# bxh1/VIDO-SLAM

Measured on AMD Instinct MI355X. Metric: frames/sec end-to-end (flow+depth+track+local-BA) at 640x480; BA iters/sec, higher is better.
Workload: dtype f32

## Files before the change

### vido-slam_amd/csrc/convsmall.hip

```cpp
#include "common.hpp"

namespace {
template <int K>
__global__ __launch_bounds__(256) void k_conv_kxk_c2(const float* __restrict__ x, const float* __restrict__ w, const float* __restrict__ bias, const float* __restrict__ res,
                                                     float* __restrict__ y, int Cin, int H, int W)
{
    constexpr int R = K / 2, TS = 16 + K - 1, CC = 8, NT = CC * TS * TS, NL = (NT + 255) / 256, NW = (CC * K * K * 2 + 255) / 256;
    __shared__ float tile[NT];
    __shared__ __attribute__((aligned(8))) float wl[NW * 256];
    const int tid = threadIdx.x, tx = tid & 15, ty = tid >> 4, bx = blockIdx.x * 16, by = blockIdx.y * 16;
    const size_t HW = (size_t)H * W;
    int toff[NL]; bool tin[NL]; int tch[NL];
#pragma unroll
    for (int j = 0; j < NL; j++) {
        const int i = min(tid + 256 * j, NT - 1), c = i / (TS * TS), r = i - c * (TS * TS), yy = r / TS, xx = r - yy * TS, gy = by + yy - R, gx = bx + xx - R;
        tch[j] = c; tin[j] = tid + 256 * j < NT && gy >= 0 && gy < H && gx >= 0 && gx < W;
        toff[j] = min(max(gy, 0), H - 1) * W + min(max(gx, 0), W - 1);
    }
    float tv[NL], wv[NW];
    auto fetch = [&](int c0) {
#pragma unroll
        for (int j = 0; j < NL; j++) { const int c = min(c0 + tch[j], Cin - 1); tv[j] = x[(size_t)c * HW + toff[j]]; }
#pragma unroll
        for (int j = 0; j < NW; j++) {
            const int i = min(tid + 256 * j, CC * K * K * 2 - 1), o = i & 1, t = (i >> 1) % (K * K), c = min(c0 + (i >> 1) / (K * K), Cin - 1);
            wv[j] = w[((size_t)o * Cin + c) * (K * K) + t];
        }
    };
    float acc0 = bias ? bias[0] : 0.f, acc1 = bias ? bias[1] : 0.f;
    fetch(0);
    for (int c0 = 0; c0 < Cin; c0 += CC) {
        __syncthreads();
#pragma unroll
        for (int j = 0; j < NL; j++) if (tid + 256 * j < NT) tile[tid + 256 * j] = (tin[j] && c0 + tch[j] < Cin) ? tv[j] : 0.f;
#pragma unroll
        for (int j = 0; j < NW; j++) { const int i = tid + 256 * j; if (i < CC * K * K * 2) wl[i] = (c0 + (i >> 1) / (K * K) < Cin) ? wv[j] : 0.f; }
        __syncthreads();
        if (c0 + CC < Cin) fetch(c0 + CC);
#pragma unroll 2
        for (int c = 0; c < CC; c++) {
            const float* tc = tile + c * TS * TS + ty * TS + tx;
            const float2* wc = (const float2*)wl + c * K * K;
#pragma unroll
            for (int dy = 0; dy < K; dy++)
#pragma unroll
                for (int dx = 0; dx < K; dx++) {
                    const float v = tc[dy * TS + dx];
                    const float2 ww = wc[dy * K + dx];
                    acc0 = fmaf(v, ww.x, acc0); acc1 = fmaf(v, ww.y, acc1);
                }
        }
    }
    const int gy = by + ty, gx = bx + tx;
    if (gy < H && gx < W) {
        const size_t o = (size_t)gy * W + gx;
        y[o] = acc0 + (res ? res[o] : 0.f); y[HW + o] = acc1 + (res ? res[HW + o] : 0.f);
    }
}

typedef float f32x16s __attribute__((ext_vector_type(16)));
template <int CB, bool RES, int D>
__global__ __launch_bounds__(256) void k_conv1x1_skinny(const float* __restrict__ x, const float* __restrict__ wp, const float* __restrict__ bias, const float* __restrict__ res,
                                                        float* __restrict__ y, int Cin, int Cout, long long HW, float slope, unsigned xbytes, unsigned wbytes)
{
    const int lane = threadIdx.x & 63, wv = __builtin_amdgcn_readfirstlane(threadIdx.x >> 6);
    const long long p0 = ((long long)blockIdx.x * 4 + wv) * 32;
    if (p0 >= HW) return;
    const long long p = min(p0 + (lane & 31), HW - 1);
    const int nkp = Cin >> 1;
    f32x16s acc[CB];
#pragma unroll
    for (int cb = 0; cb < CB; cb++)
#pragma unroll
        for (int r = 0; r < 16; r++) acc[cb][r] = 0.f;
    const __amdgpu_buffer_rsrc_t xr = __builtin_amdgcn_make_buffer_rsrc((void*)x, 0, xbytes, 0x00020000);
    const __amdgpu_buffer_rsrc_t wr = __builtin_amdgcn_make_buffer_rsrc((void*)wp, 0, wbytes, 0x00020000);
    const unsigned xvo = 4u * (unsigned)((lane >> 5) * HW + p), wvo = 4u * (unsigned)lane;
    const unsigned hw8 = 8u * (unsigned)HW;
    float b[D], a[D][CB], bn[D], an[D][CB];
    auto fetch = [&](int kp0, float (&fb)[D], float (&fa)[D][CB]) {
#pragma unroll
        for (int u = 0; u < D; u++) {
            const int kp = min(kp0 + u, nkp - 1);
            fb[u] = __builtin_bit_cast(float, __builtin_amdgcn_raw_buffer_load_b32(xr, xvo, hw8 * (unsigned)kp, 0));
#pragma unroll
            for (int cb = 0; cb < CB; cb++) fa[u][cb] = __builtin_bit_cast(float, __builtin_amdgcn_raw_buffer_load_b32(wr, wvo, 256u * (unsigned)(cb * nkp + kp), 0));
        }
    };
    constexpr bool AHEAD = D > 4;
    if (AHEAD) fetch(0, b, a);
    for (int kp0 = 0; kp0 < nkp; kp0 += D) {
        if (!AHEAD) fetch(kp0, b, a);
        else if (kp0 + D < nkp) fetch(kp0 + D, bn, an);
#pragma unroll
        for (int u = 0; u < D; u++)
            if (kp0 + u < nkp) {
#pragma unroll
                for (int cb = 0; cb < CB; cb++) acc[cb] = __builtin_amdgcn_mfma_f32_32x32x2f32(a[u][cb], b[u], acc[cb], 0, 0, 0);
            }
        if (AHEAD) {
#pragma unroll
            for (int u = 0; u < D; u++) {
                b[u] = bn[u];
#pragma unroll
                for (int cb = 0; cb < CB; cb++) a[u][cb] = an[u][cb];
            }
        }
    }
    if (p0 + (lane & 31) < HW) {
#pragma unroll
        for (int cb = 0; cb < CB; cb++) {
            float bv[16], rv[16];
#pragma unroll
            for (int r = 0; r < 16; r++) {
                const int co = min(cb * 32 + 8 * (r >> 2) + 4 * (lane >> 5) + (r & 3), Cout - 1);
                bv[r] = bias ? bias[co] : 0.f; rv[r] = RES ? res[(size_t)co * HW + p] : 0.f;
            }
#pragma unroll
            for (int r = 0; r < 16; r++) {
                const int co = cb * 32 + 8 * (r >> 2) + 4 * (lane >> 5) + (r & 3);
                const float v = acc[cb][r] + bv[r] + rv[r];
                if (co < Cout) y[(size_t)co * HW + p] = fmaxf(v, v * slope);
            }
        }
    }
}
}

extern "C" {

int vido_conv_kxk_c2(vido_ctx* ctx, const float* x, const float* w, const float* bias, const float* residual, float* y, int cin, int k, int h, int wd)
{
    if (!ctx) return VIDO_E_INVALID;
    if (!x || !w || !y || x == y || cin < 1 || h < 1 || wd < 1 || (k != 3 && k != 5 && k != 7)) return vido_set_error(ctx, VIDO_E_INVALID, "conv_kxk_c2: bad arguments (k = %d)", k);
    HIP_TRY(ctx, hipSetDevice(ctx->device));
    hipStream_t st = ctx->has_ext_stream ? ctx->ext_stream : ctx->stream;
    const dim3 grid((wd + 15) / 16, (h + 15) / 16), blk(256);
    if (k == 7) hipLaunchKernelGGL(k_conv_kxk_c2<7>, grid, blk, 0, st, x, w, bias, residual, y, cin, h, wd);
    else if (k == 5) hipLaunchKernelGGL(k_conv_kxk_c2<5>, grid, blk, 0, st, x, w, bias, residual, y, cin, h, wd);
    else hipLaunchKernelGGL(k_conv_kxk_c2<3>, grid, blk, 0, st, x, w, bias, residual, y, cin, h, wd);
    HIP_TRY(ctx, hipGetLastError());
    return VIDO_OK;
}

int vido_conv1x1_skinny(vido_ctx* ctx, const float* x, const float* w_packed, const float* bias, const float* residual, float* y, int cin, int cout, long long hw, float slope)
{
    if (!ctx) return VIDO_E_INVALID;
    if (!x || !w_packed || !y || x == y || cin < 2 || (cin & 1) || cin > 256 || cout < 1 || cout > 256 || hw < 1 || slope < 0.f || slope > 1.f || 4ll * cin * hw >= (1ll << 32))
        return vido_set_error(ctx, VIDO_E_INVALID, "conv1x1_skinny: no kernel for %d -> %d channels", cin, cout);
    HIP_TRY(ctx, hipSetDevice(ctx->device));
    hipStream_t st = ctx->has_ext_stream ? ctx->ext_stream : ctx->stream;
    const dim3 grid((unsigned)((hw + 127) / 128)), blk(256);
    const int cbn = (cout + 31) / 32;
    const unsigned xb = (unsigned)(4ll * cin * hw), wb = (unsigned)(4ll * cbn * 32 * cin);
    int depth = 16;
    if (const char* e = getenv("VIDO_SKINNY_DEPTH")) {
        depth = atoi(e);
        if (depth != 4 && depth != 8 && depth != 16) return vido_set_error(ctx, VIDO_E_INVALID, "conv1x1_skinny: VIDO_SKINNY_DEPTH=%s (4, 8 or 16)", e);
    }
#define SK_LAUNCH(CBV, DV) { if (residual) hipLaunchKernelGGL((k_conv1x1_skinny<CBV, true, DV>), grid, blk, 0, st, x, w_packed, bias, residual, y, cin, cout, hw, slope, xb, wb); \
                             else hipLaunchKernelGGL((k_conv1x1_skinny<CBV, false, DV>), grid, blk, 0, st, x, w_packed, bias, residual, y, cin, cout, hw, slope, xb, wb); }
    switch (cbn) {
    case 1: if (depth == 4) SK_LAUNCH(1, 4) else if (depth == 8) SK_LAUNCH(1, 8) else SK_LAUNCH(1, 16) break;
    case 2: SK_LAUNCH(2, 4) break; case 3: SK_LAUNCH(3, 4) break; case 4: SK_LAUNCH(4, 4) break;
    case 5: SK_LAUNCH(5, 4) break; case 6: SK_LAUNCH(6, 4) break; case 7: SK_LAUNCH(7, 4) break; default: SK_LAUNCH(8, 4) break;
    }
#undef SK_LAUNCH
    HIP_TRY(ctx, hipGetLastError());
    return VIDO_OK;
}

}
```

Baseline: 134.8.

## Add strip-tiled 2-output KxK conv and LDS-staged weights for skinny 1x1 conv

Adds a new KxK two-output-channel conv kernel in which each thread computes P horizontal pixels. It stages 64/P input channels per pass in dynamic LDS and software-pipelines row loads through a register ring, reusing window values across neighbouring pixels to cut LDS traffic. The new kernel is the default, with P=2. The skinny 1x1 MFMA conv also gains a variant that copies packed weights into LDS, used for 2-4 output blocks when the weights fit in 32 KB. It also changes the default pipeline depth to 16 or 8 for the 3- and 4-block cases, at the cost of more LDS use and register pressure.

```diff
diff --git a/vido-slam_amd/csrc/convsmall.hip b/vido-slam_amd/csrc/convsmall.hip
--- a/vido-slam_amd/csrc/convsmall.hip
+++ b/vido-slam_amd/csrc/convsmall.hip
@@ -58,12 +58,137 @@
     }
 }
 
+template <int K, int P>
+__global__ __launch_bounds__(256) void k_conv_kxk_c2_strip(const float* __restrict__ x, const float* __restrict__ w, const float* __restrict__ bias, const float* __restrict__ res,
+                                                           float* __restrict__ y, int Cin, int H, int W)
+{
+    constexpr int R = K / 2, CC = 64 / P, TW = 16 * P, TSW = TW + K - 1, TSH = 16 + K - 1, NW = TSH * TSW, NS = (NW + 255) / 256, NP = NS * 256, NV = P + K - 1;
+    constexpr int NWT = CC * K * 16, NWL = (NWT + 255) / 256, K4 = (K + 3) / 4, NB = 4, UC = 4;
+    static_assert((UC * K) % NB == 0 && NB - 1 <= K, "ring position of a row is a constant");
+    static_assert(P % 2 == 0 && TSW % 2 == 0 && NV % 2 == 0, "8-byte window reads");
+    extern __shared__ __attribute__((aligned(16))) float tile_s[];
+    float* const wl = tile_s, * const tile = tile_s + NWT;
+    const int tid = threadIdx.x, tx = tid & 15, ty = tid >> 4, bx = blockIdx.x * TW, by = blockIdx.y * 16;
+    const size_t HW = (size_t)H * W;
+    unsigned toff[NS]; bool tin[NS];
+#pragma unroll
+    for (int s = 0; s < NS; s++) {
+        const int i = min(tid + 256 * s, NW - 1), yy = i / TSW, xx = i - yy * TSW, gy = by + yy - R, gx = bx + xx - R;
+        tin[s] = tid + 256 * s < NW && gy >= 0 && gy < H && gx >= 0 && gx < W;
+        toff[s] = (unsigned)(min(max(gy, 0), H - 1) * W + min(max(gx, 0), W - 1));
+    }
+    float tv[CC][NS], wv[NWL];
+    auto fetch = [&](int c0) {
+#pragma unroll
+        for (int j = 0; j < NWL; j++) {
+            const int i = min(tid + 256 * j, NWT - 1), dx = min(i & 7, K - 1), o = (i >> 3) & 1, r = i >> 4, c = min(c0 + r / K, Cin - 1), dy = r % K;
+            wv[j] = w[((size_t)o * Cin + c) * (K * K) + dy * K + dx];
+        }
+#pragma unroll
+        for (int c = 0; c < CC; c++) {
+            const float* xc = x + (size_t)min(c0 + c, Cin - 1) * HW;
+#pragma unroll
+            for (int s = 0; s < NS; s++) tv[c][s] = xc[toff[s]];
+        }
+    };
+    float acc0[P], acc1[P];
+#pragma unroll
+    for (int p = 0; p < P; p++) { acc0[p] = bias ? bias[0] : 0.f; acc1[p] = bias ? bias[1] : 0.f; }
+    fetch(0);
+    for (int c0 = 0; c0 < Cin; c0 += CC) {
+        __syncthreads();
+#pragma unroll
+        for (int j = 0; j < NWL; j++) if (tid + 256 * j < NWT) wl[tid + 256 * j] = wv[j];
+#pragma unroll
+        for (int c = 0; c < CC; c++)
+#pragma unroll
+            for (int s = 0; s < NS; s++) tile[c * NP + tid + 256 * s] = (tin[s] && c0 + c < Cin) ? tv[c][s] : 0.f;
+        __syncthreads();
+        if (c0 + CC < Cin) fetch(c0 + CC);
+        const int nc = min(CC, Cin - c0);
+        float v[NB][NV], wa[NB][4 * K4], wb[NB][4 * K4];
+        const float* const t0 = tile + ty * TSW + tx * P;
+        auto load_row = [&](int c, int dy, float (&bv)[NV], float (&ba)[4 * K4], float (&bb)[4 * K4]) {
+            const float* tc = t0 + c * NP + dy * TSW;
+#pragma unroll
+            for (int j = 0; j < NV; j += 2) { const float2 t = *(const float2*)(tc + j); bv[j] = t.x; bv[j + 1] = t.y; }
+            const float4* wr = (const float4*)(wl + (c * K + dy) * 16);
+#pragma unroll
+            for (int q = 0; q < K4; q++) {
+                const float4 a4 = wr[q], b4 = wr[2 + q];
+                ba[4 * q] = a4.x; ba[4 * q + 1] = a4.y; ba[4 * q + 2] = a4.z; ba[4 * q + 3] = a4.w;
+                bb[4 * q] = b4.x; bb[4 * q + 1] = b4.y; bb[4 * q + 2] = b4.z; bb[4 * q + 3] = b4.w;
+            }
+        };
+        auto fma_row = [&](const float (&bv)[NV], const float (&ba)[4 * K4], const float (&bb)[4 * K4]) {
+#pragma unroll
+            for (int dx = 0; dx < K; dx++)
+#pragma unroll
+                for (int p = 0; p < P; p++) {
+                    acc0[p] = fmaf(bv[p + dx], ba[dx], acc0[p]); acc1[p] = fmaf(bv[p + dx], bb[dx], acc1[p]);
+                    asm("" : "+v"(acc0[p])); asm("" : "+v"(acc1[p]));
+                }
+        };
+        int c = 0;
+        if (nc >= UC) {
+#pragma unroll
+            for (int r = 0; r < NB - 1; r++) load_row(r / K, r % K, v[r], wa[r], wb[r]);
+            for (; c + UC <= nc; c += UC) {
+#pragma unroll
+                for (int r = 0; r < UC * K; r++) {
+                    constexpr int AH = NB - 1;
+                    load_row(min(c + (r + AH) / K, CC - 1), (r + AH) % K, v[(r + AH) % NB], wa[(r + AH) % NB], wb[(r + AH) % NB]);
+                    __builtin_amdgcn_sched_barrier(0);
+                    fma_row(v[r % NB], wa[r % NB], wb[r % NB]);
+                    __builtin_amdgcn_sched_barrier(0);
+                }
+            }
+        }
+        for (; c < nc; c++) {
+#pragma unroll
+            for (int dy = 0; dy < K; dy++) { load_row(c, dy, v[0], wa[0], wb[0]); fma_row(v[0], wa[0], wb[0]); }
+        }
+    }
+    const int gy = by + ty, gx0 = bx + tx * P;
+    if (gy < H) {
+#pragma unroll
+        for (int p = 0; p < P; p++)
+            if (gx0 + p < W) {
+                const size_t o = (size_t)gy * W + gx0 + p;
+                y[o] = acc0[p] + (res ? res[o] : 0.f); y[HW + o] = acc1[p] + (res ? res[HW + o] : 0.f);
+            }
+    }
+}
+
+constexpr int C2_STRIP_DEFAULT = 2;
+constexpr unsigned SK_WL_BYTES = 32768;
+
+template <int K, int P>
+hipError_t c2_strip_launch(int device, hipStream_t st, const float* x, const float* w, const float* bias, const float* res, float* y, int cin, int h, int wd)
+{
+    constexpr int LDS = (64 / P) * (((16 + K - 1) * (16 * P + K - 1) + 255) / 256 * 256 + K * 16) * 4;
+    static bool attr[64];
+    if (!attr[device & 63]) {
+        const hipError_t e = hipFuncSetAttribute((const void*)k_conv_kxk_c2_strip<K, P>, hipFuncAttributeMaxDynamicSharedMemorySize, LDS);
+        if (e != hipSuccess) return e;
+        attr[device & 63] = true;
+    }
+    hipLaunchKernelGGL((k_conv_kxk_c2_strip<K, P>), dim3((wd + 16 * P - 1) / (16 * P), (h + 15) / 16), dim3(256), LDS, st, x, w, bias, res, y, cin, h, wd);
+    return hipSuccess;
+}
+
 typedef float f32x16s __attribute__((ext_vector_type(16)));
-template <int CB, bool RES, int D>
+template <int CB, bool RES, int D, bool WL = false>
 __global__ __launch_bounds__(256) void k_conv1x1_skinny(const float* __restrict__ x, const float* __restrict__ wp, const float* __restrict__ bias, const float* __restrict__ res,
                                                         float* __restrict__ y, int Cin, int Cout, long long HW, float slope, unsigned xbytes, unsigned wbytes)
 {
+    extern __shared__ __attribute__((aligned(16))) float wl_s[];
     const int lane = threadIdx.x & 63, wv = __builtin_amdgcn_readfirstlane(threadIdx.x >> 6);
+    if (WL) {
+        const int n4 = CB * (Cin >> 1) * 16;
+        for (int i = threadIdx.x; i < n4; i += 256) ((float4*)wl_s)[i] = ((const float4*)wp)[i];
+        __syncthreads();
+    }
     const long long p0 = ((long long)blockIdx.x * 4 + wv) * 32;
     if (p0 >= HW) return;
     const long long p = min(p0 + (lane & 31), HW - 1);
@@ -83,8 +208,10 @@
         for (int u = 0; u < D; u++) {
             const int kp = min(kp0 + u, nkp - 1);
             fb[u] = __builtin_bit_cast(float, __builtin_amdgcn_raw_buffer_load_b32(xr, xvo, hw8 * (unsigned)kp, 0));
-#pragma unroll
-            for (int cb = 0; cb < CB; cb++) fa[u][cb] = __builtin_bit_cast(float, __builtin_amdgcn_raw_buffer_load_b32(wr, wvo, 256u * (unsigned)(cb * nkp + kp), 0));
+            if (!WL) {
+#pragma unroll
+                for (int cb = 0; cb < CB; cb++) fa[u][cb] = __builtin_bit_cast(float, __builtin_amdgcn_raw_buffer_load_b32(wr, wvo, 256u * (unsigned)(cb * nkp + kp), 0));
+            }
         }
     };
     constexpr bool AHEAD = D > 4;
@@ -96,14 +223,16 @@
         for (int u = 0; u < D; u++)
             if (kp0 + u < nkp) {
 #pragma unroll
-                for (int cb = 0; cb < CB; cb++) acc[cb] = __builtin_amdgcn_mfma_f32_32x32x2f32(a[u][cb], b[u], acc[cb], 0, 0, 0);
+                for (int cb = 0; cb < CB; cb++) acc[cb] = __builtin_amdgcn_mfma_f32_32x32x2f32(WL ? wl_s[(cb * nkp + kp0 + u) * 64 + lane] : a[u][cb], b[u], acc[cb], 0, 0, 0);
             }
         if (AHEAD) {
 #pragma unroll
             for (int u = 0; u < D; u++) {
                 b[u] = bn[u];
-#pragma unroll
-                for (int cb = 0; cb < CB; cb++) a[u][cb] = an[u][cb];
+                if (!WL) {
+#pragma unroll
+                    for (int cb = 0; cb < CB; cb++) a[u][cb] = an[u][cb];
+                }
             }
         }
     }
@@ -135,10 +264,23 @@
     if (!x || !w || !y || x == y || cin < 1 || h < 1 || wd < 1 || (k != 3 && k != 5 && k != 7)) return vido_set_error(ctx, VIDO_E_INVALID, "conv_kxk_c2: bad arguments (k = %d)", k);
     HIP_TRY(ctx, hipSetDevice(ctx->device));
     hipStream_t st = ctx->has_ext_stream ? ctx->ext_stream : ctx->stream;
-    const dim3 grid((wd + 15) / 16, (h + 15) / 16), blk(256);
-    if (k == 7) hipLaunchKernelGGL(k_conv_kxk_c2<7>, grid, blk, 0, st, x, w, bias, residual, y, cin, h, wd);
-    else if (k == 5) hipLaunchKernelGGL(k_conv_kxk_c2<5>, grid, blk, 0, st, x, w, bias, residual, y, cin, h, wd);
-    else hipLaunchKernelGGL(k_conv_kxk_c2<3>, grid, blk, 0, st, x, w, bias, residual, y, cin, h, wd);
+    int strip = C2_STRIP_DEFAULT;
+    if (const char* e = getenv("VIDO_C2_STRIP")) {
+        strip = atoi(e);
+        if (strip != 1 && strip != 2 && strip != 4 && strip != 8) return vido_set_error(ctx, VIDO_E_INVALID, "conv_kxk_c2: VIDO_C2_STRIP=%s (1, 2, 4 or 8)", e);
+    }
+    if (strip == 1) {
+        const dim3 grid((wd + 15) / 16, (h + 15) / 16), blk(256);
+        if (k == 7) hipLaunchKernelGGL(k_conv_kxk_c2<7>, grid, blk, 0, st, x, w, bias, residual, y, cin, h, wd);
+        else if (k == 5) hipLaunchKernelGGL(k_conv_kxk_c2<5>, grid, blk, 0, st, x, w, bias, residual, y, cin, h, wd);
+        else hipLaunchKernelGGL(k_conv_kxk_c2<3>, grid, blk, 0, st, x, w, bias, residual, y, cin, h, wd);
+    } else {
+#define C2_STRIP(KV) HIP_TRY(ctx, strip == 2 ? (c2_strip_launch<KV, 2>)(ctx->device, st, x, w, bias, residual, y, cin, h, wd) \
+                                : strip == 4 ? (c2_strip_launch<KV, 4>)(ctx->device, st, x, w, bias, residual, y, cin, h, wd) \
+                                             : (c2_strip_launch<KV, 8>)(ctx->device, st, x, w, bias, residual, y, cin, h, wd))
+        if (k == 7) C2_STRIP(7); else if (k == 5) C2_STRIP(5); else C2_STRIP(3);
+#undef C2_STRIP
+    }
     HIP_TRY(ctx, hipGetLastError());
     return VIDO_OK;
 }
@@ -154,15 +296,22 @@
     const int cbn = (cout + 31) / 32;
     const unsigned xb = (unsigned)(4ll * cin * hw), wb = (unsigned)(4ll * cbn * 32 * cin);
     int depth = 16;
+    bool named = false;
     if (const char* e = getenv("VIDO_SKINNY_DEPTH")) {
-        depth = atoi(e);
+        depth = atoi(e); named = true;
         if (depth != 4 && depth != 8 && depth != 16) return vido_set_error(ctx, VIDO_E_INVALID, "conv1x1_skinny: VIDO_SKINNY_DEPTH=%s (4, 8 or 16)", e);
     }
 #define SK_LAUNCH(CBV, DV) { if (residual) hipLaunchKernelGGL((k_conv1x1_skinny<CBV, true, DV>), grid, blk, 0, st, x, w_packed, bias, residual, y, cin, cout, hw, slope, xb, wb); \
                              else hipLaunchKernelGGL((k_conv1x1_skinny<CBV, false, DV>), grid, blk, 0, st, x, w_packed, bias, residual, y, cin, cout, hw, slope, xb, wb); }
     switch (cbn) {
     case 1: if (depth == 4) SK_LAUNCH(1, 4) else if (depth == 8) SK_LAUNCH(1, 8) else SK_LAUNCH(1, 16) break;
-    case 2: SK_LAUNCH(2, 4) break; case 3: SK_LAUNCH(3, 4) break; case 4: SK_LAUNCH(4, 4) break;
+#define SK_LAUNCH_WL(CBV, DV) { if (residual) hipLaunchKernelGGL((k_conv1x1_skinny<CBV, true, DV, true>), grid, blk, wb, st, x, w_packed, bias, residual, y, cin, cout, hw, slope, xb, wb); \
+                                else hipLaunchKernelGGL((k_conv1x1_skinny<CBV, false, DV, true>), grid, blk, wb, st, x, w_packed, bias, residual, y, cin, cout, hw, slope, xb, wb); }
+#define SK_WIDE(CBV, DG) if (depth == 4) SK_LAUNCH(CBV, 4) else if (wb <= SK_WL_BYTES) { if (depth == 8) SK_LAUNCH_WL(CBV, 8) else SK_LAUNCH_WL(CBV, 16) } \
+                         else if (depth == 8) SK_LAUNCH(CBV, 8) else SK_LAUNCH(CBV, DG)
+    case 2: if (!named) SK_LAUNCH(2, 4) else SK_WIDE(2, 16) break; case 3: SK_WIDE(3, 8) break; case 4: SK_WIDE(4, 8) break;
+#undef SK_WIDE
+#undef SK_LAUNCH_WL
     case 5: SK_LAUNCH(5, 4) break; case 6: SK_LAUNCH(6, 4) break; case 7: SK_LAUNCH(7, 4) break; default: SK_LAUNCH(8, 4) break;
     }
 #undef SK_LAUNCH
```

Result: no change. 136.2 (median of 6 runs) (+1.0%).
